# HKUST-Aerial-Robotics/FIESTA

Hardware: AMD Instinct MI355X
Metric: esdf_updated_voxels_per_sec (higher is better)
Workload: dtype u32

## Files before the change

### fiesta_amd/csrc/dense_map.hip

```cpp
#include "dense_map.hpp"
#include "checkpoint.hpp"
#include "frontier_kernels.hpp"
#include "ray_query_kernels.hpp"
#include "reach_kernels.hpp"
#include "reach_matrix_kernels.hpp"
#include "corridor_kernels.hpp"
#include "view_kernels.hpp"
#include "ft_kernels.hpp"
#include "nn_kernels.hpp"
#include "mask_kernels.hpp"
#include "level_kernels.hpp"
#include "path_cost_kernels.hpp"
#include "refine_kernels.hpp"
#include "timing_kernels.hpp"
#include "path_kernels.hpp"
#include "relax_kernels.hpp"

#include <algorithm>
#include <chrono>
#include <cmath>
#include <cstdlib>
#include <cstring>

namespace fiesta {
// ... 1603 lines not shown
  for (int attempt = 0; attempt < 2; ++attempt) {
    cells = attempt == 0 && cells_wanted() && run_cells(st, 0, false);
    if (!cells) {
      bool exact = true;
      if (!run_bulk(st, 0, &exact)) return false;
    }
    const unsigned long long *failed = cells ? &counters_[C_NN_FAILED] : nullptr;
    MaskArgs a = ma;
    a.failed = failed;
    FIESTA_HIP_CHECK(hipEventRecord(ev_cert, stream_));
    hipLaunchKernelGGL(k_mask_classify, dim3(classify_blocks), dim3(256), 0, stream_, a);
    #ifndef FIESTA_WALK_PARTS
#define FIESTA_WALK_PARTS 32
#endif
    hipLaunchKernelGGL(k_mask_walk, dim3(kMaskSegs * FIESTA_WALK_PARTS), dim3(256), 0, stream_, a);
    hipLaunchKernelGGL(k_mask_cells, dim3(std::min(classify_blocks, 1024)), dim3(256), 0, stream_, a);
    FIESTA_HIP_CHECK(hipGetLastError());
    FIESTA_HIP_CHECK(hipEventRecord(ev_rep, stream_));
    gi = 0;
    chain = std::min(std::max(mask_chain_hint_, 2), kMaskIters);
    launch_chain(chain, failed);
    FIESTA_HIP_CHECK(hipEventRecord(ev_end, stream_));
    FIESTA_HIP_CHECK(hipMemcpyAsync(h_mask_ctr_, mask_ctr_, MC_SEG0 * sizeof(unsigned long long), hipMemcpyDeviceToHost, stream_));
    if (cells) FIESTA_HIP_CHECK(hipMemcpyAsync(&h_counters_[C_FT_OVF0], &counters_[C_FT_OVF0], 7 * sizeof(unsigned long long), hipMemcpyDeviceToHost, stream_));
    FIESTA_HIP_CHECK(hipStreamSynchronize(stream_));
#if defined(FIESTA_PROBE)
    fprintf(stderr, "PROBE walks %llu: straight n-sum %llu, steps %llu | paths %llu, positions loaded %llu, refused by cell %llu, n-sum %llu | entries %llu, candidates %llu, none %llu, certified %llu\n",
            h_mask_ctr_[MC_WALKS], h_mask_ctr_[MC_CHANGED0 + 12], h_mask_ctr_[MC_CHANGED0 + 13], h_mask_ctr_[MC_CHANGED0 + 14], h_mask_ctr_[MC_CHANGED0 + 15],
            h_mask_ctr_[MC_CHANGED0 + 16], h_mask_ctr_[MC_CHANGED0 + 17], h_mask_ctr_[MC_CHANGED0 + 18], h_mask_ctr_[MC_CHANGED0 + 19], h_mask_ctr_[MC_CHANGED0 + 20],
            h_mask_ctr_[MC_CHANGED0 + 21]);
#endif
    if (!cells || h_counters_[C_NN_FAILED] == 0) {
      if (cells) nn_fail_streak_ = 0;
      break;
    }
    nn_fail_streak_ = std::min(nn_fail_streak_ + 1, 6);
    nn_skip_ = 4 << nn_fail_streak_;
    const int64_t nfailed = (int64_t)h_counters_[C_NN_FAILED];
    reset_stats_counters(true);
    if (st) {
      memset(&st->cells, 0, sizeof(st->cells));
      st->nn_failed = nfailed;
    }
  }
  float m1 = 0, m2 = 0, m3 = 0, mc = 0, mr = 0;
  (void)hipEventElapsedTime(&m1, ft_ev_[0], ft_ev_[1]);
  (void)hipEventElapsedTime(&m2, ft_ev_[1], ft_ev_[2]);
  (void)hipEventElapsedTime(&m3, ft_ev_[2], ft_ev_[3]);
  (void)hipEventElapsedTime(&mc, ev_cert, ev_rep);
  (void)hipEventElapsedTime(&mr, ev_rep, ev_end);
  if (st)
    for (int k = 0; k < 8; ++k) st->prof[k] = (int64_t)h_mask_ctr_[MC_CHANGED0 + k];
  if (h_mask_ctr_[MC_OVERFLOW] != 0) {
    if (mask_seg_cap_ * kMaskSegs >= (size_t)g.n) return false;
    mask_seg_cap_ *= 2;
    tr_occ_ = nullptr, tr_out_ = nullptr, tr_cellobs_ = nullptr;
    reset_stats_counters(true);
    return run_masked(st);
  }
  int total_iters = 0;
  for (int n = chain;;) {
    int k = 0;
    while (k < n && h_mask_ctr_[MC_CHANGED0 + k] != 0) ++k;
    total_iters += k < n ? k + 1 : n;
    if (k < n || h_mask_ctr_[MC_QUADS] == 0) break;
    FIESTA_HIP_CHECK(hipMemsetAsync(&mask_ctr_[MC_CHANGED0], 0, kMaskIters * sizeof(unsigned long long), stream_));
    FIESTA_HIP_CHECK(hipEventRecord(ev_rep, stream_));
    n = 4;
    launch_chain(n, nullptr);
    FIESTA_HIP_CHECK(hipEventRecord(ev_end, stream_));
    FIESTA_HIP_CHECK(hipMemcpyAsync(&h_mask_ctr_[MC_CHANGED0], &mask_ctr_[MC_CHANGED0], kMaskIters * sizeof(unsigned long long), hipMemcpyDeviceToHost, stream_));
    FIESTA_HIP_CHECK(hipStreamSynchronize(stream_));
    float more = 0;
    (void)hipEventElapsedTime(&more, ev_rep, ev_end);
    mr += more;
  }
  mask_chain_hint_ = std::min(total_iters + 1, kMaskIters);
  std::swap(coc_, mask_out_.p);
  zero_counters(C_INSERT, 2);
  host_counts_[0] = host_counts_[1] = 0;
  queues_zeroed_ = false;
  if (track_) {
    zero_counter(C_MAXD2);
    hipLaunchKernelGGL(k_maxd2_scan, dim3(grid_for(g_.n, 256, 4096)), dim3(256), 0, stream_, g_, (const vox_t *)coc_, counters_);
    FIESTA_HIP_CHECK(hipGetLastError());
  }
  FIESTA_HIP_CHECK(hipEventRecord(ev1_, stream_));
  FIESTA_HIP_CHECK(hipEventSynchronize(ev1_));
  h_counters_fresh_ = false;
  if (cells) nn_last_ms_ = (double)m1 + m2 + m3, nn_last_nocc_ = (long long)h_counters_[C_NOCC];
  else ft_last_ms_ = (double)m1 + m2 + m3;
  if (st) {
    float ms = 0;
    FIESTA_HIP_CHECK(hipEventElapsedTime(&ms, ev0_, ev1_));
    st->device_ms = ms;
    st->bulk = 1, st->cells = cells ? 1 : 0, st->masked = 1;
    if (cells) {
      st->nn_cells_ms = m1, st->nn_lists_ms = m2, st->nn_fill_ms = m3;
      st->nn_entries = (int64_t)h_counters_[C_NN_ENTRIES];
    } else {
      st->ft_rows_ms = m1, st->ft_plane_ms = m2, st->ft_x_ms = m3;
    }
    st->mask_certify_ms = mc, st->mask_repair_ms = mr;
    st->mask_uncertified = (int64_t)h_mask_ctr_[MC_MARKED], st->mask_iterations = total_iters, st->mask_walks = (int64_t)h_mask_ctr_[MC_WALKS];
    st->mask_quads = (int64_t)h_mask_ctr_[MC_QUADS];
    st->relax_ms = (double)m1 + m2 + m3 + mc + mr;
    st->relax_launches = 3 + 3 + 2 * total_iters;
  }
  return true;
}

struct HostMs {
  fiesta_hip_stats *st;
  std::chrono::steady_clock::time_point h0 = std::chrono::steady_clock::now();
  ~HostMs() { if (st) st->host_ms = std::chrono::duration<double, std::milli>(std::chrono::steady_clock::now() - h0).count(); }
};

void DenseMap::bulk_finish(fiesta_hip_stats *st, bool cells, bool published) {
  static_assert(C_DELETE == C_INSERT + 1, "counter layout");
  nn_clean_ = false;
  if (published) {
    FIESTA_HIP_CHECK(hipEventRecord(ev1_, stream_));
    FIESTA_HIP_CHECK(hipEventSynchronize(ev1_));
    published = h_counters_[C_NN_CURSOR] == nn_tag_;
    if (published) {
      h_counters_fresh_ = false;
      if (h_counters_[C_NN_FAILED] == 0) {
        queues_zeroed_ = false;
        host_counts_[0] = host_counts_[1] = 0;
        nn_clean_ = true;
      }
    }
  }
  if (!published) {
    if (!queues_zeroed_) zero_counters(C_INSERT, 2);
    queues_zeroed_ = false;
    host_counts_[0] = host_counts_[1] = 0;
    if (g_.sharded) zero_counter(C_REMOTE_DEL);
    FIESTA_HIP_CHECK(hipEventRecord(ev1_, stream_));
    collect_stats(nullptr);
    FIESTA_HIP_CHECK(hipEventSynchronize(ev1_));
  }
  float m1 = 0, m2 = 0, m3 = 0;
  const bool timed = hipEventElapsedTime(&m1, ft_ev_[0], ft_ev_[1]) == hipSuccess && hipEventElapsedTime(&m2, ft_ev_[1], ft_ev_[2]) == hipSuccess &&
                     hipEventElapsedTime(&m3, ft_ev_[2], ft_ev_[3]) == hipSuccess;
  if (st) {
    float ms = 0;
    FIESTA_HIP_CHECK(hipEventElapsedTime(&ms, ev0_, ev1_));
    st->device_ms = ms;
    if (cells) {
      st->nn_cells_ms = m1, st->nn_lists_ms = m2, st->nn_fill_ms = m3;
      st->nn_entries = (int64_t)h_counters_[C_NN_ENTRIES];
      st->nn_failed = (int64_t)h_counters_[C_NN_FAILED];
      if (st->nn_incremental) st->nn_dirty_cells = (int64_t)h_counters_[C_NN_DIRTY];
      else st->nn_brute_cells = (int64_t)h_counters_[C_NN_BRUTE];
    } else {
      st->ft_rows_ms = m1, st->ft_plane_ms = m2, st->ft_x_ms = m3;
      st->ft_overflow[0] = (int64_t)h_counters_[C_FT_OVF0], st->ft_overflow[3] = (int64_t)h_counters_[C_FT_OVF0 + 3];
    }
    st->relax_ms = (double)m1 + m2 + m3;
  }
  if (cells && published && !(st && st->nn_incremental)) nn_last_brute_ = (long long)h_counters_[C_NN_BRUTE];
  if (timed) {
    if (cells) {
      if (h_counters_[C_NN_FAILED] == 0) nn_last_ms_ = (double)m1 + m2 + m3, nn_last_nocc_ = (long long)h_counters_[C_NOCC];
    } else {
      ft_last_ms_ = (double)m1 + m2 + m3;
    }
  }
}

bool DenseMap::bulk_try(fiesta_hip_stats *st, int margin, bool *exact) {
  ++field_epoch_;
  use_device();
  nn_clean_ = false;
  nn_valid_ = false;
  ++epoch_;
  FIESTA_HIP_CHECK(hipEventRecord(ev0_, stream_));
  reset_stats_counters();
  if (st) memset(st, 0, sizeof(*st));
  tried_cells_ = false;
  if (cells_wanted() && run_cells(st, margin, false)) {
    FIESTA_HIP_CHECK(hipMemcpyAsync(&h_counters_[C_FT_OVF0], &counters_[C_FT_OVF0], 7 * sizeof(unsigned long long), hipMemcpyDeviceToHost, stream_));
    FIESTA_HIP_CHECK(hipStreamSynchronize(stream_));
    if (h_counters_[C_NN_FAILED] == 0) {
      nn_fail_streak_ = 0;
      tried_cells_ = true;
      if (exact) *exact = true;
      if (st) st->ft_max_d2 = (int64_t)h_counters_[C_FT_MAXD2];
      return true;
    }
    cells_back_off();
    const int64_t failed = (int64_t)h_counters_[C_NN_FAILED];
    reset_stats_counters();
    if (st) {
      memset(st, 0, sizeof(*st));
      st->nn_failed = failed;
    }
  }
  return run_bulk(st, margin, exact);
}
void DenseMap::bulk_commit(fiesta_hip_stats *st) {
  ++field_epoch_;
  use_device();
  if (!ft_in_place_) std::swap(coc_, ft_out_.p);
  HostMs host_ms{st};
  bulk_finish(st, tried_cells_);
}
void DenseMap::bulk_probe(unsigned long long *ni, unsigned long long *nd, long long *nocc, bool *eligible) {
  use_device();
  FIESTA_HIP_CHECK(hipMemcpyAsync(&h_counters_[C_INSERT], &counters_[C_INSERT], 4 * sizeof(unsigned long long),
                                  hipMemcpyDeviceToHost, stream_));
  FIESTA_HIP_CHECK(hipStreamSynchronize(stream_));
  for (int k = 0; k < 4; ++k) host_counts_[k] = h_counters_[C_INSERT + k];
  host_counts_valid_ = true;
  *ni = h_counters_[C_INSERT], *nd = h_counters_[C_DELETE];
  *nocc = (long long)h_counters_[C_NOCC];
  *eligible = bulk_eligible(*ni, *nd);
}

void DenseMap::level_tuning(int grid_groups, long long spin_limit) { LevelEngine::tuning(lv_, grid_groups, spin_limit); }
int DenseMap::level_trace(uint32_t *out48) const { return LevelEngine::trace(lv_, out48); }

bool DenseMap::run_levels(fiesta_hip_stats *st, unsigned long long ni, unsigned long long nd) {
  if (!lv_) {
    lv_ = new LevelEngine;
#ifdef FIESTA_HIP_TUNING
    if (const char *e = getenv("FIESTA_HIP_GRID_ENTER")) lv_->grid_enter = (uint32_t)atoi(e);
    if (const char *e = getenv("FIESTA_HIP_GRID_MIN")) lv_->grid_min = (uint32_t)atoi(e);
#endif
  }
  const uint32_t want = update_engine_ == 3 ? (uint32_t)std::min<int64_t>(std::max<int64_t>(g_.n / 4, 1 << 20), 1 << 26) : (1u << 20);
  lv_->ensure(want, stream_);
  LevelUpdate u{};
  u.stream = stream_, u.t0 = ev0_;
  u.coc = coc_, u.counters = counters_, u.track = track_;
  u.ins = (const uint32_t *)ins_.p, u.ni = ni;
  u.scan = nd != 0, u.full_window = g_.full_window();
  u.pinned = update_engine_ == 3, u.tiny = ni + nd <= (unsigned long long)LevelEngine::kTiny;
  u.nwords = g_.n;
  u.tg = TileGrid{tx_, ty_, ntx_, nty_, ntz_}, u.tile_flag = tile_flag_[0], u.tile_list = tile_list_[0], u.list_count = &counters_[C_LIST0];
  const int bounded = (track_ && nd) ? 1 : 0;
  const auto scan = [&](bool levels, const LevelArgs &a) {
    if (levels && bounded) hipLaunchKernelGGL(k_del_bbox, dim3(1), dim3(1024), 0, stream_, g_, (const uint32_t *)del_.p, (int64_t)nd, counters_);
    hipLaunchKernelGGL(levels ? k_invalidate<true> : k_invalidate<false>, dim3((grid_for(g_.n / 16 + 1, 256, 4096) + 7) / 8 * 8), dim3(256), 0,
                       stream_, g_, u.tg, coc_, (const uint32_t *)occbits_, (const uint32_t *)gocc_, tile_flag_[0], tile_list_[0],
                       &counters_[C_LIST0], counters_, bounded, a);
    FIESTA_HIP_CHECK(hipGetLastError());
  };
  host_counts_[0] = host_counts_[1] = 0;
  if (!lv_->update(DenseSpace{g_, occbits_, lv_box(g_)}, u, scan, st)) return false;
  h_counters_fresh_ = false;
  if (st) st->device_ms = st->relax_ms;
  return true;
}

bool DenseMap::serve_by_transform(fiesta_hip_stats *st, unsigned long long ni, unsigned long long nd, bool nn_was_clean, bool nn_was_valid) {
  const bool want_cells = cells_wanted();
  const bool lean = want_cells && nn_was_clean;
  if (lean) {
    queues_zeroed_ = false;
    ft_counters_clean_ = true;
  } else {
    queues_zeroed_ = !g_.sharded && g_.nx <= 2048 && g_.ny <= 2048 && g_.nz <= 2048;
    reset_stats_counters(true, queues_zeroed_);
  }
  const int64_t ncells8 = (int64_t)((g_.nx + 7) / 8) * ((g_.ny + 7) / 8) * ((g_.nz + 7) / 8);
  if (want_cells && nn_was_valid && !g_.wrap && (int64_t)(ni + nd) * 180 <= ncells8 / 2 && run_cells(st, 0, true, true, ni, nd)) {
    bulk_finish(st, true, true);
    if (h_counters_[C_NN_FAILED] == 0) {
      nn_fail_streak_ = 0;
      nn_valid_ = true;
      return true;
    }
    notes_ |= FIESTA_HIP_NOTE_INCREMENTAL_REDONE;
    FIESTA_HIP_CHECK(hipMemsetAsync(nn_dirty_flag_.p, 0, nn_dirty_flag_.cap * sizeof(uint32_t), stream_));
    if (st) memset(&st->cells, 0, sizeof(st->cells)), st->nn_incremental = 0;
    restart_attempt();
  }
  if (want_cells && run_cells(st, 0, true)) {
    bulk_finish(st, true, true);
    if (h_counters_[C_NN_FAILED] == 0) {
      nn_fail_streak_ = 0;
      nn_valid_ = !g_.sharded && h_counters_[C_NN_SPARSE] == 0;
      return true;
    }
    cells_back_off();
    notes_ |= FIESTA_HIP_NOTE_CELLS_FAILED;
    const int64_t failed = (int64_t)h_counters_[C_NN_FAILED];
    if (st) {
      memset(&st->cells, 0, sizeof(st->cells));
      st->nn_failed = failed;
    }
    restart_attempt();
  }
  bool exact = true;
  if (run_bulk(st, 0, &exact)) {
    bulk_finish(st);
    return true;
  }
  if (queues_zeroed_) {
    h_counters_[C_INSERT] = ni, h_counters_[C_DELETE] = nd;
    FIESTA_HIP_CHECK(hipMemcpyAsync(&counters_[C_INSERT], &h_counters_[C_INSERT], 2 * sizeof(unsigned long long), hipMemcpyHostToDevice, stream_));
    queues_zeroed_ = false;
  }
  return false;
// ... 871 lines not shown
```

### fiesta_amd/csrc/nn_kernels.hpp

```cpp
#pragma once
#include "common.hpp"
#include "nn_core.hpp"

namespace fiesta {

struct NnArgs {
  nn::Geom g;
  const uint8_t *cellobs;
  const uint32_t *occ;
  int sx0, sy0, szb;
  int sny, snzw;
  uint32_t *ctab;
  uint32_t *sites;
  uint32_t sites_cap;
  uint32_t *lists;
  unsigned long long *cursor;
  unsigned long long *failed;
  unsigned long long *entries;
  unsigned long long *maxd2;
  vox_t *coc;
  uint32_t *dump;
  unsigned long long *pub, *queues, *track_dst;
  unsigned long long tag;
  int pub_failed, pub_entries, pub_maxd2, pub_tag, pub_dirty, pub_brute, pub_sparse;
// ... 216 lines not shown
    if (rank == 0) (void)atomicExch(counter, 0u);
    __builtin_amdgcn_fence(__ATOMIC_ACQ_REL, "wavefront");
  }
  __device__ __forceinline__ int slot() { return (int)atomicAdd(counter, 1u); }
  __device__ __forceinline__ int count_now() const { return (int)min(atomicAdd(counter, 0u), (uint32_t)nn::kRaw); }
  __device__ __forceinline__ void put(int k, uint32_t v) { raw[k] = v; }
  __device__ __forceinline__ uint32_t get(int k) const { return raw[k]; }
  __device__ __forceinline__ int count() const {
    __builtin_amdgcn_fence(__ATOMIC_ACQ_REL, "wavefront");
    return (int)atomicAdd(counter, 0u);
  }
};

template <bool WRAP>
__global__ __launch_bounds__(1024) __attribute__((amdgpu_waves_per_eu(8, 8))) void k_nn_lists(NnArgs a) {
  __shared__ uint16_t s_tab[kStageNR * kStageNZ];
  __shared__ uint32_t s_first[kStageNR], s_soff[kStageNR], s_cnt[kStageNR];
  __shared__ uint32_t s_sites[kStageSites];
  __shared__ uint32_t s_slots[256];
  __shared__ uint32_t s_raw[256 * (nn::kRaw + 1)];
  __shared__ uint32_t s_total, s_bad, s_sum, s_done;
  __shared__ uint32_t s_te2[256], s_tw[256], s_bin[8];
  __shared__ uint16_t s_order[256];
  __shared__ uint8_t s_key[256];
  const nn::Geom &g = a.g;
  if (*a.failed) return;
  const int tid = (int)threadIdx.x;
  const int cz0 = g.lz0 + (int)blockIdx.x * 64, cy0 = g.ly0 + (int)blockIdx.y * 4, cx = g.lx0 + (int)blockIdx.z;
  const int X0 = cx - kStageK, Y0 = cy0 - kStageK, Zf = cz0 - kStageK;
  const nn::Frame fr = nn::frame_of(g);
  const int64_t rowlen = g.ncz + 1;
  if (tid < 256) s_slots[tid] = 0;
  if (tid == 0) s_bad = 0, s_sum = 0, s_done = 0;
  if (tid < 8) s_bin[tid] = 0;
  if (tid < kStageNR) {
    const int X = X0 + tid / kStageNY, Y = Y0 + tid % kStageNY;
    uint32_t f = 0, l = 0;
    if ((unsigned)X < (unsigned)g.ncx && (unsigned)Y < (unsigned)g.ncy) {
      const uint32_t *row = a.ctab + ((int64_t)X * g.ncy + Y) * rowlen;
      f = row[min(max(Zf, 0), g.ncz)], l = row[min(max(Zf + kStageNZ - 1, 0), g.ncz)];
    }
    s_first[tid] = f, s_cnt[tid] = l - f;
  }
  __syncthreads();
  if (tid < 64) {
    const uint32_t c0 = tid < kStageNR ? s_cnt[tid] : 0u, c1 = tid + 64 < kStageNR ? s_cnt[tid + 64] : 0u;
    uint32_t i0 = c0, i1 = c1;
    for (int off = 1; off < 64; off <<= 1) {
      const uint32_t u0 = (uint32_t)__shfl_up((int)i0, off), u1 = (uint32_t)__shfl_up((int)i1, off);
      if (tid >= off) i0 += u0, i1 += u1;
    }
    const uint32_t t0 = (uint32_t)__shfl((int)i0, 63);
    if (tid < kStageNR) s_soff[tid] = i0 - c0;
    if (tid + 64 < kStageNR) s_soff[tid + 64] = t0 + i1 - c1;
    if (tid == 63) s_total = t0 + i1;
  }
  __syncthreads();
  const bool staged = s_total <= (uint32_t)kStageSites;
  if (staged) {
    for (int idx = tid; idx < kStageNR * kStageNZ; idx += 1024) {
      const int row = idx / kStageNZ, e = idx - row * kStageNZ;
      const int X = X0 + row / kStageNY, Y = Y0 + row % kStageNY;
      uint32_t v = 0;
      if ((unsigned)X < (unsigned)g.ncx && (unsigned)Y < (unsigned)g.ncy)
        v = a.ctab[((int64_t)X * g.ncy + Y) * rowlen + min(max(Zf + e, 0), g.ncz)] - s_first[row];
      s_tab[idx] = (uint16_t)v;
    }
    for (int idx = tid; idx < kStageNR * 16; idx += 1024) {
      const int row = idx >> 4;
      const uint32_t cnt = s_cnt[row], first = s_first[row], at = s_soff[row];
      for (uint32_t j = (uint32_t)(idx & 15); j < cnt; j += 16) s_sites[at + j] = a.sites[first + j];
    }
  }
  __syncthreads();
  const int team_i = tid >> 2;
  QuadTeam team{tid & 3, &s_slots[team_i], &s_raw[team_i * (nn::kRaw + 1)]};
  const StagedSrcT<WRAP> ssrc{staged ? s_tab : nullptr, s_soff, s_sites, -(X0 * kStageNY + Y0), -Zf};
  {
    const int cz = cz0 + (team_i & 63), cy = cy0 + (team_i >> 6);
    const bool live = cz < g.lz1 && cy < g.ly1 && !(a.cellobs && a.cellobs[((int64_t)cx * g.ncy + cy) * g.ncz + cz] == 0);
    int te2 = nn::kNone, key = 7;
    uint32_t tw = 0xFFFFFFFFu;
    if (live) {
      if (staged) nn::first_competitor(ssrc, team, cx, cy, cz, nn::kKfirst, te2, tw);
      key = min(nn::window_reach<WRAP>(te2, tw, cx, cy, cz), 6);
    }
    if (team.rank == 0) {
      s_te2[team_i] = (uint32_t)te2, s_tw[team_i] = tw, s_key[team_i] = (uint8_t)key;
      atomicAdd(&s_bin[key], 1u);
    }
  }
  __syncthreads();
  if (tid == 0) {
    uint32_t at = 0;
    for (int k = 0; k < 8; ++k) {
      const uint32_t c = s_bin[k];
      s_bin[k] = at, at += c;
    }
  }
  __syncthreads();
  if (tid < 256) s_order[atomicAdd(&s_bin[s_key[tid]], 1u)] = (uint16_t)tid;
  __syncthreads();
  const int ci = s_order[team_i];
  const int cz = cz0 + (ci & 63), cy = cy0 + (ci >> 6);
  int n = 0;
  bool live = cz < g.lz1 && cy < g.ly1;
  if (live && a.cellobs && a.cellobs[((int64_t)cx * g.ncy + cy) * g.ncz + cz] == 0) {
    live = false;
    if (team.rank == 0) a.lists[(((int64_t)cx * g.ncy + cy) * g.ncz + cz) * nn::kStride] = 0u;
  }
  if (live) {
    const int64_t cell = ((int64_t)cx * g.ncy + cy) * g.ncz + cz;
    uint32_t *rec = a.lists + cell * nn::kStride;
    n = -1;
    if (staged) n = nn::build_list(ssrc, team, cx, cy, cz, rec, true, (int)s_te2[ci], s_tw[ci], fr);
    if (n < 0) {
      const HybridSrcT<WRAP> src{ssrc, nn::PlainSrcT<WRAP>{a.ctab, a.sites, g.ncx, g.ncy, g.ncz}, X0, Y0, Zf};
      n = nn::build_list(src, team, cx, cy, cz, rec, false, nn::kNone, 0xFFFFFFFFu, fr);
    }
  }
  bool hard = live && team.rank == 0 && n == 0;
  if (hard && a.fail_list && fr.open == 0 && *a.nfail < a.fail_cap) {
    const unsigned long long at = atomicAdd(a.nfail, 1ull);
    if (at < a.fail_cap) {
      a.fail_list[at] = (uint32_t)(((int64_t)cx * g.ncy + cy) * g.ncz + cz);
      hard = false;
    }
  }
  const unsigned long long bad = __ballot(hard);
  int sum = (live && team.rank == 0) ? n : 0;
  for (int off = 32; off > 0; off >>= 1) sum += __shfl_xor(sum, off);
  if ((tid & 63) == 0) {
    if (bad) atomicAdd(&s_bad, (uint32_t)__popcll(bad));
    if (sum) atomicAdd(&s_sum, (uint32_t)sum);
    __threadfence_block();
    if (atomicAdd(&s_done, 1u) == 15u) {
      const uint32_t b = atomicAdd(&s_bad, 0u), t = atomicAdd(&s_sum, 0u);
      if (b) atomicAdd(a.failed, (unsigned long long)b);
      if (t) atomicAdd(a.entries, (unsigned long long)t);
    }
  }
}

__device__ __forceinline__ void nn_dot4_pair(uint32_t a, uint32_t b0, uint32_t b1, int &d0, int &d1) {
  asm("v_dot4_i32_i8 %0, %2, %3, 0\n\tv_dot4_i32_i8 %1, %2, %4, 0\n\ts_nop 2" : "=&v"(d0), "=&v"(d1) : "v"(a), "v"(b0), "v"(b1));
}

#ifndef FIESTA_FILL_BLOCKS
#define FIESTA_FILL_BLOCKS 16384
#endif
constexpr int kFillBlocks = FIESTA_FILL_BLOCKS;
constexpr int kListPad = 256;

template <bool TRACK, bool OFFSET = false>
__global__ __launch_bounds__(256) void k_nn_fill_full(NnArgs a) {
  constexpr int kTileRow = 40;
  __shared__ __attribute__((aligned(16))) uint32_t land[4][2][nn::kStride];
  __shared__ __attribute__((aligned(16))) uint32_t tile[4][nn::kB * kTileRow];
  const nn::Geom &g = a.g;
  if (*a.failed) return;
  const int lane = threadIdx.x & 63, wave = __builtin_amdgcn_readfirstlane((int)(threadIdx.x >> 6));
  const int quads = OFFSET ? (g.lz1 - g.lz0 + 3) >> 2 : g.ncz >> 2;
  const int rows_y = OFFSET ? g.ly1 - g.ly0 : g.ncy;
  const uint32_t nq = (uint32_t)((OFFSET ? g.lx1 - g.lx0 : g.ncx) * rows_y) * (uint32_t)quads;
  const uint32_t per = OFFSET ? (nq + gridDim.x * 4u - 1u) / (gridDim.x * 4u) : nq / (gridDim.x * 4u);
  const uint32_t q0 = (blockIdx.x * 4u + (uint32_t)wave) * per, q1 = OFFSET ? min(q0 + per, nq) : q0 + per;
  if (OFFSET && q0 >= q1) return;
  const int row0 = (int)(q0 / (uint32_t)quads);
  const int y = lane >> 3, z = lane & 7;
  const uint32_t ayz = (uint32_t)y | ((uint32_t)z << 8);
  const int64_t plane = (int64_t)g.ny * g.nz;
  const int loff4 = y * g.nz + 4 * z;
  uint32_t dmax = 0;
  const uint32_t zone0 = (uint32_t)(size_t)&land[wave][0][0];
  uint32_t *const mytile = &tile[wave][0];
  struct At { int cx, cy, q; };
  auto fetch = [&](const At &c, const int cell_of_quad, const int zone) {
    const int64_t cell = OFFSET ? ((int64_t)(g.lx0 + c.cx) * g.ncy + (g.ly0 + c.cy)) * g.ncz + min(g.lz0 + 4 * c.q + cell_of_quad, g.lz1 - 1)
                                : ((int64_t)c.cx * g.ncy + c.cy) * g.ncz + 4 * c.q + cell_of_quad;
    const uint32_t *lp = a.lists + cell * nn::kStride + lane, *hp = lp + 64;
    const uint32_t at = zone0 + (uint32_t)zone * (uint32_t)(nn::kStride * 4);
    asm volatile("s_mov_b32 m0, %0\n\tglobal_load_lds_dword %1, off\n\t"
                 "s_mov_b32 m0, %2\n\tglobal_load_lds_dword %3, off"
                 : : "s"(at), "v"(lp), "s"(at + 256u), "v"(hp) : "memory", "m0");
  };
  auto advance = [&](At &c) {
    if (++c.q == quads) {
      c.q = 0;
      if (++c.cy == rows_y) c.cy = 0, ++c.cx;
    }
  };
  auto serve = [&](const int zone, uint32_t *ww, const bool col_in, const int xin_lo, const int xin_hi) {
    const uint32_t *lz = &land[wave][zone][0];
    const int cnt = __builtin_amdgcn_readfirstlane((int)lz[0]);
    uint32_t best[nn::kB];
#pragma unroll
    for (int x = 0; x < nn::kB; ++x) best[x] = 0xFFFFFFFFu;
    for (int i = 0; i < cnt; i += 2) {
      const uint4 e0 = *reinterpret_cast<const uint4 *>(lz + 4 + 4 * i), e1 = *reinterpret_cast<const uint4 *>(lz + 8 + 4 * i);
      int d0, d1;
      nn_dot4_pair(ayz, e0.x, e1.x, d0, d1);
      uint32_t k0 = ((uint32_t)d0 << nn::kSH) + e0.y, k1 = ((uint32_t)d1 << nn::kSH) + e1.y;
      best[0] = min(best[0], min(k0, k1));
#pragma unroll
      for (int x = 1; x < nn::kB; ++x) {
        k0 += e0.z, k1 += e1.z;
        best[x] = min(best[x], min(k0, k1));
      }
    }
#pragma unroll
    for (int x = 0; x < nn::kB; ++x) {
      ww[x] = *reinterpret_cast<const uint32_t *>(reinterpret_cast<const char *>(lz + 7) + (best[x] & 0x1F0u));
      if (TRACK && (!OFFSET || (col_in && x >= xin_lo && x < xin_hi)))
        dmax = max(dmax, (best[x] >> nn::kSH) - (uint32_t)nn::kBias + (uint32_t)(x * x + y * y + z * z));
    }
  };
  At c{row0 / rows_y, row0 % rows_y, (int)(q0 % (uint32_t)quads)};
  fetch(c, 0, 0);
  asm volatile("s_waitcnt vmcnt(0)" ::: "memory");
  for (uint32_t q = q0; q < q1; ++q) {
    uint32_t ww[4][nn::kB];
    At nxt = c;
    if (q + 1 < q1) advance(nxt);
#pragma unroll
    for (int k = 0; k < 4; ++k) {
      if (k < 3) fetch(c, k + 1, (k + 1) & 1); else fetch(nxt, 0, 0);
      if (k == 0) {
        if (OFFSET) asm volatile("s_waitcnt vmcnt(18)" ::: "memory");
        else asm volatile("s_waitcnt vmcnt(10)" ::: "memory");
      } else {
        asm volatile("s_waitcnt vmcnt(2)" ::: "memory");
      }
      bool col_in = true;
      int xin_lo = 0, xin_hi = nn::kB;
      if (OFFSET && TRACK) {
        const int cz = g.lz0 + 4 * c.q + k;
        const int Y = nn::kB * (g.ly0 + c.cy) + y - g.fy, Z = nn::kB * cz + z - g.fz, X0 = nn::kB * (g.lx0 + c.cx) - g.fx;
        col_in = cz < g.lz1 && (unsigned)Y < (unsigned)g.ay && (unsigned)Z < (unsigned)g.az;
        xin_lo = max(0, -X0), xin_hi = min(nn::kB, g.ax - X0);
      }
      serve(k & 1, ww[k], col_in, xin_lo, xin_hi);
      asm volatile("s_waitcnt lgkmcnt(0)" ::: "memory");
    }
    if (!OFFSET) {
      vox_t *slab = a.coc + ((int64_t)(nn::kB * c.cx) * g.ny + nn::kB * c.cy) * g.nz + 4 * nn::kB * c.q;
#pragma unroll
      for (int x = 0; x < nn::kB; ++x) {
#pragma unroll
        for (int k = 0; k < 4; ++k) mytile[y * kTileRow + nn::kB * k + z] = ww[k][x];
        const uint4 v = *reinterpret_cast<const uint4 *>(&mytile[y * kTileRow + 4 * z]);
        *reinterpret_cast<uint4 *>(slab + loff4) = v;
        slab += plane;
      }
    } else {
      const int srow = lane >> 4, spair = lane & 15;
      const int X0 = nn::kB * (g.lx0 + c.cx) - g.fx, Y0 = nn::kB * (g.ly0 + c.cy) - g.fy;
      const int Zq = nn::kB * (g.lz0 + 4 * c.q) + 2 * spair;
      const bool zin = (unsigned)(Zq - g.fz) < (unsigned)g.az && Zq < nn::kB * g.lz1;
      const int64_t aplane = (int64_t)g.ay * g.az;
      uint32_t *const mydump = a.dump + 2 * lane;
#pragma unroll
      for (int x = 0; x < nn::kB; ++x) {
#pragma unroll
        for (int k = 0; k < 4; ++k) mytile[y * kTileRow + nn::kB * k + z] = ww[k][x];
        const bool xin = (unsigned)(X0 + x) < (unsigned)g.ax;
#pragma unroll
        for (int h = 0; h < 2; ++h) {
          const int r = srow + 4 * h;
          const uint2 v = *reinterpret_cast<const uint2 *>(&mytile[r * kTileRow + 2 * spair]);
          const bool in = xin && zin && (unsigned)(Y0 + r) < (unsigned)g.ay;
          uint32_t *dst = in ? a.coc + (int64_t)(X0 + x) * aplane + (int64_t)(Y0 + r) * g.az + (Zq - g.fz) : mydump;
          *reinterpret_cast<uint2 *>(dst) = v;
        }
      }
    }
    c = nxt;
  }
  if (TRACK) {
    for (int off = 32; off > 0; off >>= 1) dmax = max(dmax, (uint32_t)__shfl_xor((int)dmax, off));
    if (lane == 0 && (unsigned long long)dmax > *a.maxd2) atomicMax(a.maxd2, (unsigned long long)dmax);
  }
}

typedef __attribute__((address_space(4))) const uint32_t nn_cu32;
typedef uint32_t nn_u32x4 __attribute__((ext_vector_type(4)));
typedef __attribute__((address_space(4))) const nn_u32x4 nn_cu32x4;
template <bool TRACK>
__device__ __forceinline__ void nn_fill_cell(const NnArgs &a, const int cx, const int cy, const int cz, const int lane, uint32_t &dmax) {
  const nn::Geom &g = a.g;
  const int64_t cell = ((int64_t)cx * g.ncy + cy) * g.ncz + cz;
  const uint32_t *rec = a.lists + cell * nn::kStride;
  nn_cu32 *lp = reinterpret_cast<nn_cu32 *>(reinterpret_cast<uintptr_t>(rec));
  const int cnt = (int)lp[0];
  const int y = lane >> 3, z = lane & 7;
  const uint32_t ayz = (uint32_t)y | ((uint32_t)z << 8);
  uint32_t best[nn::kB];
#pragma unroll
  for (int x = 0; x < nn::kB; ++x) best[x] = 0xFFFFFFFFu;
  for (int i = 0; i < cnt; ++i) {
    const nn_u32x4 e = *reinterpret_cast<nn_cu32x4 *>(lp + 4 + 4 * i);
    uint32_t k = ((uint32_t)__builtin_amdgcn_sdot4((int)ayz, (int)e.x, 0, false) << nn::kSH) + e.y;
    best[0] = min(best[0], k);
#pragma unroll
    for (int x = 1; x < nn::kB; ++x) {
      k += e.z;
      best[x] = min(best[x], k);
    }
  }
  const int X0 = nn::kB * cx - g.fx, Y = nn::kB * cy + y - g.fy, Z = nn::kB * cz + z - g.fz;
  const bool inyz = (unsigned)Y < (unsigned)g.ay && (unsigned)Z < (unsigned)g.az;
  vox_t *out = a.coc + ((int64_t)X0 * g.ay + Y) * g.az + Z;
  const int64_t plane = (int64_t)g.ay * g.az;
#pragma unroll
  for (int x = 0; x < nn::kB; ++x) {
    const uint32_t ww = rec[7 + ((best[x] & 0x1F0u) >> 2)];
    if (inyz && (unsigned)(X0 + x) < (unsigned)g.ax) {
      out[x * plane] = ww;
      if (TRACK) dmax = max(dmax, (best[x] >> nn::kSH) - (uint32_t)nn::kBias + (uint32_t)(x * x + y * y + z * z));
    }
  }
}

template <bool TRACK>
__global__ __launch_bounds__(256) void k_nn_fill(NnArgs a) {
  const nn::Geom &g = a.g;
  if (*a.failed) return;
  const int lane = threadIdx.x & 63, wave = __builtin_amdgcn_readfirstlane((int)(threadIdx.x >> 6));
  const int cz = g.lz0 + (int)blockIdx.x * 4 + wave, cy = g.ly0 + (int)blockIdx.y, cx = g.lx0 + (int)blockIdx.z;
  if (cz >= g.lz1) return;
  uint32_t dmax = 0;
  nn_fill_cell<TRACK>(a, cx, cy, cz, lane, dmax);
  if (TRACK) {
    for (int off = 32; off > 0; off >>= 1) dmax = max(dmax, (uint32_t)__shfl_xor((int)dmax, off));
    if (lane == 0 && (unsigned long long)dmax > *a.maxd2) atomicMax(a.maxd2, (unsigned long long)dmax);
  }
}

constexpr int kMarkQueue = 4096;
__global__ __launch_bounds__(1024) void k_nn_mark(NnArgs a) {
  __shared__ uint32_t s_q[kMarkQueue];
  __shared__ uint32_t s_n;
  __shared__ unsigned long long s_base;
  const nn::Geom &g = a.g;
  const uint32_t total = a.nchg[0] + a.nchg[1];
  constexpr int E = 2 * nn::kKmax + 1, E3 = E * E * E;
  const unsigned long long pairs = (unsigned long long)total * E3;
  if (threadIdx.x == 0) s_n = 0;
  __syncthreads();
  for (unsigned long long p0 = (unsigned long long)blockIdx.x * blockDim.x; p0 < pairs; p0 += (unsigned long long)gridDim.x * blockDim.x) {
    const unsigned long long p = p0 + threadIdx.x;
    if (p < pairs) {
      const uint32_t v = (uint32_t)(p / E3);
      const int o = (int)(p - (unsigned long long)v * E3);
      const uint32_t idx = v < a.nchg[0] ? a.chg[0][v] : a.chg[1][v - a.nchg[0]];
      const int z = (int)(idx % (uint32_t)g.nz), y = (int)((idx / (uint32_t)g.nz) % (uint32_t)g.ny), x = (int)(idx / ((uint32_t)g.nz * (uint32_t)g.ny));
      const int dz = o % E - nn::kKmax, dy = (o / E) % E - nn::kKmax, dx = o / (E * E) - nn::kKmax;
      const int cx = (x >> 3) + dx, cy = (y >> 3) + dy, cz = (z >> 3) + dz;
      if ((unsigned)cx < (unsigned)g.ncx && (unsigned)cy < (unsigned)g.ncy && (unsigned)cz < (unsigned)g.ncz) {
        const int64_t c = ((int64_t)cx * g.ncy + cy) * g.ncz + cz;
        const int r = max(max(dx < 0 ? -dx : dx, dy < 0 ? -dy : dy), dz < 0 ? -dz : dz);
        if (r <= (int)(a.lists[c * nn::kStride + 1] & 255u) && a.dirty_flag[c] == 0u && atomicExch(&a.dirty_flag[c], 1u) == 0u)
          s_q[atomicAdd(&s_n, 1u)] = (uint32_t)c;
      }
    }
    __syncthreads();
    const uint32_t n = s_n;
    const bool last = p0 + (unsigned long long)gridDim.x * blockDim.x >= pairs;
    if (n && (last || n > (uint32_t)kMarkQueue - 1024u)) {
      if (threadIdx.x == 0) s_base = atomicAdd(a.dirty_count, (unsigned long long)n);
      __syncthreads();
      const unsigned long long base = s_base;
      for (uint32_t i = threadIdx.x; i < n; i += blockDim.x)
        if (base + i < a.dirty_cap) a.dirty_list[base + i] = s_q[i];
      __syncthreads();
      if (threadIdx.x == 0) s_n = 0;
    }
    __syncthreads();
  }
}

__global__ __launch_bounds__(256) void k_nn_lists_dirty(NnArgs a) {
  __shared__ uint32_t s_slots[16];
  __shared__ uint32_t s_raw[16 * (nn::kRaw + 1)];
  const nn::Geom &g = a.g;
  if (*a.failed) return;
  const unsigned long long nd = *a.dirty_count;
  if (nd > a.dirty_cap) {
    if (blockIdx.x == 0 && threadIdx.x == 0) atomicAdd(a.failed, 1ull);
    return;
  }
  const int tid = (int)threadIdx.x, team_i = tid >> 4;
  const nn::Frame fr = nn::frame_of(g);
  const nn::PlainSrcT<false> src{a.ctab, a.sites, g.ncx, g.ncy, g.ncz};
  unsigned bad = 0, entries = 0;
  for (unsigned long long i = blockIdx.x * 16ull + (unsigned long long)team_i; i < nd; i += gridDim.x * 16ull) {
    const uint32_t c = a.dirty_list[i];
    const int cz = (int)(c % (uint32_t)g.ncz), cy = (int)((c / (uint32_t)g.ncz) % (uint32_t)g.ncy), cx = (int)(c / ((uint32_t)g.ncz * (uint32_t)g.ncy));
    WideTeam team{tid & 15, &s_slots[team_i], &s_raw[team_i * (nn::kRaw + 1)]};
    if (team.rank == 0) s_slots[team_i] = 0;
    __builtin_amdgcn_fence(__ATOMIC_ACQ_REL, "wavefront");
    const int n = nn::build_list(src, team, cx, cy, cz, a.lists + (int64_t)c * nn::kStride, false, nn::kNone, 0xFFFFFFFFu, fr);
    if (team.rank == 0) {
      if (n <= 0) ++bad; else entries += (unsigned)n;
    }
  }
  for (int off = 32; off > 0; off >>= 1) {
    bad += (unsigned)__shfl_xor((int)bad, off);
    entries += (unsigned)__shfl_xor((int)entries, off);
  }
  if ((tid & 63) == 0) {
    if (bad) atomicAdd(a.failed, (unsigned long long)bad);
    (void)entries;
  }
}

template <bool TRACK>
__global__ __launch_bounds__(256) void k_nn_fill_dirty(NnArgs a) {
  const nn::Geom &g = a.g;
  if (*a.failed) return;
  const unsigned long long nd = *a.dirty_count;
  const int lane = threadIdx.x & 63, wave = __builtin_amdgcn_readfirstlane((int)(threadIdx.x >> 6));
  uint32_t dmax = 0;
  for (unsigned long long i = blockIdx.x * 4ull + (unsigned long long)wave; i < nd; i += gridDim.x * 4ull) {
    const uint32_t c = a.dirty_list[i];
    const int cz = (int)(c % (uint32_t)g.ncz), cy = (int)((c / (uint32_t)g.ncz) % (uint32_t)g.ncy), cx = (int)(c / ((uint32_t)g.ncz * (uint32_t)g.ncy));
    nn_fill_cell<TRACK>(a, cx, cy, cz, lane, dmax);
    if (lane == 0) a.dirty_flag[c] = 0u;
  }
  if (TRACK) {
    for (int off = 32; off > 0; off >>= 1) dmax = max(dmax, (uint32_t)__shfl_xor((int)dmax, off));
    if (lane == 0 && (unsigned long long)dmax > *a.maxd2) atomicMax(a.maxd2, (unsigned long long)dmax);
  }
}

// ... 104 lines not shown
```

Before: 8.038 billion.

## Fetch NN list records by count-sized lines instead of whole records in fill

Splits the non-offset full fill kernel into a separate path that loads each cell's candidate list into LDS in 128-byte lines. The first line of all four cells in a quad is prefetched one quad ahead, a second line is fetched only when the count exceeds 7, and the whole record is loaded synchronously only when it exceeds 15. The aim is to cut global-to-LDS traffic for cells with short lists. In exchange it adds count-dependent branching, a serialized wait on the rare long-list path, and a second LDS buffer per wave. It also records the tracked max d2 in stats for the NN path.

```diff
diff --git a/fiesta_amd/csrc/dense_map.hip b/fiesta_amd/csrc/dense_map.hip
--- a/fiesta_amd/csrc/dense_map.hip
+++ b/fiesta_amd/csrc/dense_map.hip
@@ -1779,6 +1779,7 @@
       st->nn_cells_ms = m1, st->nn_lists_ms = m2, st->nn_fill_ms = m3;
       st->nn_entries = (int64_t)h_counters_[C_NN_ENTRIES];
       st->nn_failed = (int64_t)h_counters_[C_NN_FAILED];
+      if (published && track_) st->ft_max_d2 = (int64_t)h_counters_[C_FT_MAXD2];
       if (st->nn_incremental) st->nn_dirty_cells = (int64_t)h_counters_[C_NN_DIRTY];
       else st->nn_brute_cells = (int64_t)h_counters_[C_NN_BRUTE];
     } else {
diff --git a/fiesta_amd/csrc/nn_kernels.hpp b/fiesta_amd/csrc/nn_kernels.hpp
--- a/fiesta_amd/csrc/nn_kernels.hpp
+++ b/fiesta_amd/csrc/nn_kernels.hpp
@@ -392,32 +392,149 @@
 constexpr int kFillBlocks = FIESTA_FILL_BLOCKS;
 constexpr int kListPad = 256;
 
-template <bool TRACK, bool OFFSET = false>
-__global__ __launch_bounds__(256) void k_nn_fill_full(NnArgs a) {
+template <bool TRACK>
+__device__ __forceinline__ void nn_fill_full_lines(const NnArgs &a) {
   constexpr int kTileRow = 40;
-  __shared__ __attribute__((aligned(16))) uint32_t land[4][2][nn::kStride];
+  constexpr int kSlot = 64;
+  __shared__ __attribute__((aligned(16))) uint32_t land[4][2][4][kSlot];
+  __shared__ __attribute__((aligned(16))) uint32_t whole[4][nn::kStride];
   __shared__ __attribute__((aligned(16))) uint32_t tile[4][nn::kB * kTileRow];
   const nn::Geom &g = a.g;
   if (*a.failed) return;
   const int lane = threadIdx.x & 63, wave = __builtin_amdgcn_readfirstlane((int)(threadIdx.x >> 6));
-  const int quads = OFFSET ? (g.lz1 - g.lz0 + 3) >> 2 : g.ncz >> 2;
-  const int rows_y = OFFSET ? g.ly1 - g.ly0 : g.ncy;
-  const uint32_t nq = (uint32_t)((OFFSET ? g.lx1 - g.lx0 : g.ncx) * rows_y) * (uint32_t)quads;
-  const uint32_t per = OFFSET ? (nq + gridDim.x * 4u - 1u) / (gridDim.x * 4u) : nq / (gridDim.x * 4u);
-  const uint32_t q0 = (blockIdx.x * 4u + (uint32_t)wave) * per, q1 = OFFSET ? min(q0 + per, nq) : q0 + per;
-  if (OFFSET && q0 >= q1) return;
+  const int quads = g.ncz >> 2;
+  const uint32_t nq = (uint32_t)(g.ncx * g.ncy) * (uint32_t)quads;
+  const uint32_t per = nq / (gridDim.x * 4u);
+  const uint32_t q0 = (uint32_t)__builtin_amdgcn_readfirstlane((int)((blockIdx.x * 4u + (uint32_t)wave) * per)), q1 = q0 + per;
   const int row0 = (int)(q0 / (uint32_t)quads);
   const int y = lane >> 3, z = lane & 7;
   const uint32_t ayz = (uint32_t)y | ((uint32_t)z << 8);
   const int64_t plane = (int64_t)g.ny * g.nz;
   const int loff4 = y * g.nz + 4 * z;
+  const uint32_t lane4 = 4u * (uint32_t)lane;
+  uint32_t dmax = 0;
+  const uint32_t set0 = (uint32_t)(size_t)&land[wave][0][0][0];
+  const uint32_t whole0 = (uint32_t)(size_t)&whole[wave][0];
+  uint32_t *const mytile = &tile[wave][0];
+  const char *const recs = reinterpret_cast<const char *>(a.lists);
+  auto quad_recs = [&](const uint32_t q) { return recs + (uint64_t)q * (uint64_t)(4 * nn::kStride * 4); };
+  auto fetch_lines = [&](const char *p0, const char *p1, const char *p2, const char *p3, const uint32_t at) {
+    if (lane < 32)
+      asm volatile("s_mov_b32 m0, %5\n\ts_nop 0\n\tglobal_load_lds_dword %0, %1\n\t"
+                   "s_mov_b32 m0, %6\n\ts_nop 0\n\tglobal_load_lds_dword %0, %2\n\t"
+                   "s_mov_b32 m0, %7\n\ts_nop 0\n\tglobal_load_lds_dword %0, %3\n\t"
+                   "s_mov_b32 m0, %8\n\ts_nop 0\n\tglobal_load_lds_dword %0, %4"
+                   : : "v"(lane4), "s"(p0), "s"(p1), "s"(p2), "s"(p3), "s"(at), "s"(at + 256u), "s"(at + 512u), "s"(at + 768u)
+                   : "memory", "m0");
+  };
+  auto fetch_line0 = [&](const char *qr, const int set) {
+    fetch_lines(qr, qr + 512, qr + 1024, qr + 1536, set0 + (uint32_t)set * (uint32_t)(4 * kSlot * 4));
+  };
+  auto fetch_line1 = [&](const char *qr, const int set, const int *cnt) {
+    fetch_lines(qr + (cnt[0] > 7 ? 128 : 0), qr + 512 + (cnt[1] > 7 ? 128 : 0), qr + 1024 + (cnt[2] > 7 ? 128 : 0),
+                qr + 1536 + (cnt[3] > 7 ? 128 : 0), set0 + (uint32_t)set * (uint32_t)(4 * kSlot * 4) + 128u);
+  };
+  auto fetch_whole = [&](const char *qr, const int k) {
+    asm volatile("s_mov_b32 m0, %3\n\ts_nop 0\n\tglobal_load_lds_dword %0, %1\n\t"
+                 "s_mov_b32 m0, %4\n\ts_nop 0\n\tglobal_load_lds_dword %0, %2\n\t"
+                 "s_waitcnt vmcnt(0)"
+                 : : "v"(lane4), "s"(qr + 512 * k), "s"(qr + 512 * k + 256), "s"(whole0), "s"(whole0 + 256u) : "memory", "m0");
+  };
+  auto serve = [&](const uint32_t *lz, const int cnt, uint32_t *ww) {
+    uint32_t best[nn::kB];
+#pragma unroll
+    for (int x = 0; x < nn::kB; ++x) best[x] = 0xFFFFFFFFu;
+    for (int i = 0; i < cnt; i += 2) {
+      const int j = i + 1 < cnt ? i + 1 : i;
+      const uint4 e0 = *reinterpret_cast<const uint4 *>(lz + 4 + 4 * i), e1 = *reinterpret_cast<const uint4 *>(lz + 4 + 4 * j);
+      int d0, d1;
+      nn_dot4_pair(ayz, e0.x, e1.x, d0, d1);
+      uint32_t k0 = ((uint32_t)d0 << nn::kSH) + e0.y, k1 = ((uint32_t)d1 << nn::kSH) + e1.y;
+      best[0] = min(best[0], min(k0, k1));
+#pragma unroll
+      for (int x = 1; x < nn::kB; ++x) {
+        k0 += e0.z, k1 += e1.z;
+        best[x] = min(best[x], min(k0, k1));
+      }
+    }
+#pragma unroll
+    for (int x = 0; x < nn::kB; ++x) {
+      ww[x] = *reinterpret_cast<const uint32_t *>(reinterpret_cast<const char *>(lz + 7) + (best[x] & 0x1F0u));
+      if (TRACK) dmax = max(dmax, (best[x] >> nn::kSH) - (uint32_t)nn::kBias + (uint32_t)(x * x + y * y + z * z));
+    }
+  };
+  struct At { int cx, cy, q; };
+  At c{row0 / g.ncy, row0 % g.ncy, (int)(q0 % (uint32_t)quads)};
+  fetch_line0(quad_recs(q0), 0);
+  for (uint32_t q = q0; q < q1; ++q) {
+    if (q == q0) asm volatile("s_waitcnt vmcnt(0)" ::: "memory");
+    else asm volatile("s_waitcnt vmcnt(8)" ::: "memory");
+    const int set = (int)((q - q0) & 1u);
+    const uint32_t *const slots = &land[wave][set][0][0];
+    const char *const qr = quad_recs(q);
+    int cnt[4];
+#pragma unroll
+    for (int k = 0; k < 4; ++k)
+      cnt[k] = min(__builtin_amdgcn_readfirstlane((int)slots[k * kSlot]), nn::kCap);
+    asm volatile("s_waitcnt lgkmcnt(0)" ::: "memory");
+    fetch_line1(qr, set, cnt);
+    fetch_line0(quad_recs(q + 1 < q1 ? q + 1 : q), set ^ 1);
+    uint32_t ww[4][nn::kB];
+#pragma unroll
+    for (int k = 0; k < 4; ++k) {
+      const uint32_t *lz = slots + k * kSlot;
+      if (cnt[k] > 15) {
+        fetch_whole(qr, k);
+        lz = &whole[wave][0];
+      } else if (cnt[k] > 7) {
+        asm volatile("s_waitcnt vmcnt(4)" ::: "memory");
+      }
+      serve(lz, cnt[k], ww[k]);
+      asm volatile("s_waitcnt lgkmcnt(0)" ::: "memory");
+    }
+    vox_t *slab = a.coc + ((int64_t)(nn::kB * c.cx) * g.ny + nn::kB * c.cy) * g.nz + 4 * nn::kB * c.q;
+#pragma unroll
+    for (int x = 0; x < nn::kB; ++x) {
+#pragma unroll
+      for (int k = 0; k < 4; ++k) mytile[y * kTileRow + nn::kB * k + z] = ww[k][x];
+      const uint4 v = *reinterpret_cast<const uint4 *>(&mytile[y * kTileRow + 4 * z]);
+      *reinterpret_cast<uint4 *>(slab + loff4) = v;
+      slab += plane;
+    }
+    if (++c.q == quads) {
+      c.q = 0;
+      if (++c.cy == g.ncy) c.cy = 0, ++c.cx;
+    }
+  }
+  if (TRACK) {
+    for (int off = 32; off > 0; off >>= 1) dmax = max(dmax, (uint32_t)__shfl_xor((int)dmax, off));
+    if (lane == 0 && (unsigned long long)dmax > *a.maxd2) atomicMax(a.maxd2, (unsigned long long)dmax);
+  }
+}
+
+template <bool TRACK>
+__device__ __forceinline__ void nn_fill_full_offset(const NnArgs &a) {
+  constexpr int kTileRow = 40;
+  __shared__ __attribute__((aligned(16))) uint32_t land[4][2][nn::kStride];
+  __shared__ __attribute__((aligned(16))) uint32_t tile[4][nn::kB * kTileRow];
+  const nn::Geom &g = a.g;
+  if (*a.failed) return;
+  const int lane = threadIdx.x & 63, wave = __builtin_amdgcn_readfirstlane((int)(threadIdx.x >> 6));
+  const int quads = (g.lz1 - g.lz0 + 3) >> 2;
+  const int rows_y = g.ly1 - g.ly0;
+  const uint32_t nq = (uint32_t)((g.lx1 - g.lx0) * rows_y) * (uint32_t)quads;
+  const uint32_t per = (nq + gridDim.x * 4u - 1u) / (gridDim.x * 4u);
+  const uint32_t q0 = (blockIdx.x * 4u + (uint32_t)wave) * per, q1 = min(q0 + per, nq);
+  if (q0 >= q1) return;
+  const int row0 = (int)(q0 / (uint32_t)quads);
+  const int y = lane >> 3, z = lane & 7;
+  const uint32_t ayz = (uint32_t)y | ((uint32_t)z << 8);
   uint32_t dmax = 0;
   const uint32_t zone0 = (uint32_t)(size_t)&land[wave][0][0];
   uint32_t *const mytile = &tile[wave][0];
   struct At { int cx, cy, q; };
   auto fetch = [&](const At &c, const int cell_of_quad, const int zone) {
-    const int64_t cell = OFFSET ? ((int64_t)(g.lx0 + c.cx) * g.ncy + (g.ly0 + c.cy)) * g.ncz + min(g.lz0 + 4 * c.q + cell_of_quad, g.lz1 - 1)
-                                : ((int64_t)c.cx * g.ncy + c.cy) * g.ncz + 4 * c.q + cell_of_quad;
+    const int64_t cell = ((int64_t)(g.lx0 + c.cx) * g.ncy + (g.ly0 + c.cy)) * g.ncz + min(g.lz0 + 4 * c.q + cell_of_quad, g.lz1 - 1);
     const uint32_t *lp = a.lists + cell * nn::kStride + lane, *hp = lp + 64;
     const uint32_t at = zone0 + (uint32_t)zone * (uint32_t)(nn::kStride * 4);
     asm volatile("s_mov_b32 m0, %0\n\tglobal_load_lds_dword %1, off\n\t"
@@ -451,7 +568,7 @@
 #pragma unroll
     for (int x = 0; x < nn::kB; ++x) {
       ww[x] = *reinterpret_cast<const uint32_t *>(reinterpret_cast<const char *>(lz + 7) + (best[x] & 0x1F0u));
-      if (TRACK && (!OFFSET || (col_in && x >= xin_lo && x < xin_hi)))
+      if (TRACK && col_in && x >= xin_lo && x < xin_hi)
         dmax = max(dmax, (best[x] >> nn::kSH) - (uint32_t)nn::kBias + (uint32_t)(x * x + y * y + z * z));
     }
   };
@@ -465,15 +582,11 @@
 #pragma unroll
     for (int k = 0; k < 4; ++k) {
       if (k < 3) fetch(c, k + 1, (k + 1) & 1); else fetch(nxt, 0, 0);
-      if (k == 0) {
-        if (OFFSET) asm volatile("s_waitcnt vmcnt(18)" ::: "memory");
-        else asm volatile("s_waitcnt vmcnt(10)" ::: "memory");
-      } else {
-        asm volatile("s_waitcnt vmcnt(2)" ::: "memory");
-      }
+      if (k == 0) asm volatile("s_waitcnt vmcnt(18)" ::: "memory");
+      else asm volatile("s_waitcnt vmcnt(2)" ::: "memory");
       bool col_in = true;
       int xin_lo = 0, xin_hi = nn::kB;
-      if (OFFSET && TRACK) {
+      if (TRACK) {
         const int cz = g.lz0 + 4 * c.q + k;
         const int Y = nn::kB * (g.ly0 + c.cy) + y - g.fy, Z = nn::kB * cz + z - g.fz, X0 = nn::kB * (g.lx0 + c.cx) - g.fx;
         col_in = cz < g.lz1 && (unsigned)Y < (unsigned)g.ay && (unsigned)Z < (unsigned)g.az;
@@ -482,36 +595,24 @@
       serve(k & 1, ww[k], col_in, xin_lo, xin_hi);
       asm volatile("s_waitcnt lgkmcnt(0)" ::: "memory");
     }
-    if (!OFFSET) {
-      vox_t *slab = a.coc + ((int64_t)(nn::kB * c.cx) * g.ny + nn::kB * c.cy) * g.nz + 4 * nn::kB * c.q;
-#pragma unroll
-      for (int x = 0; x < nn::kB; ++x) {
-#pragma unroll
-        for (int k = 0; k < 4; ++k) mytile[y * kTileRow + nn::kB * k + z] = ww[k][x];
-        const uint4 v = *reinterpret_cast<const uint4 *>(&mytile[y * kTileRow + 4 * z]);
-        *reinterpret_cast<uint4 *>(slab + loff4) = v;
-        slab += plane;
-      }
-    } else {
-      const int srow = lane >> 4, spair = lane & 15;
-      const int X0 = nn::kB * (g.lx0 + c.cx) - g.fx, Y0 = nn::kB * (g.ly0 + c.cy) - g.fy;
-      const int Zq = nn::kB * (g.lz0 + 4 * c.q) + 2 * spair;
-      const bool zin = (unsigned)(Zq - g.fz) < (unsigned)g.az && Zq < nn::kB * g.lz1;
-      const int64_t aplane = (int64_t)g.ay * g.az;
-      uint32_t *const mydump = a.dump + 2 * lane;
-#pragma unroll
-      for (int x = 0; x < nn::kB; ++x) {
-#pragma unroll
-        for (int k = 0; k < 4; ++k) mytile[y * kTileRow + nn::kB * k + z] = ww[k][x];
-        const bool xin = (unsigned)(X0 + x) < (unsigned)g.ax;
-#pragma unroll
-        for (int h = 0; h < 2; ++h) {
-          const int r = srow + 4 * h;
-          const uint2 v = *reinterpret_cast<const uint2 *>(&mytile[r * kTileRow + 2 * spair]);
-          const bool in = xin && zin && (unsigned)(Y0 + r) < (unsigned)g.ay;
-          uint32_t *dst = in ? a.coc + (int64_t)(X0 + x) * aplane + (int64_t)(Y0 + r) * g.az + (Zq - g.fz) : mydump;
-          *reinterpret_cast<uint2 *>(dst) = v;
-        }
+    const int srow = lane >> 4, spair = lane & 15;
+    const int X0 = nn::kB * (g.lx0 + c.cx) - g.fx, Y0 = nn::kB * (g.ly0 + c.cy) - g.fy;
+    const int Zq = nn::kB * (g.lz0 + 4 * c.q) + 2 * spair;
+    const bool zin = (unsigned)(Zq - g.fz) < (unsigned)g.az && Zq < nn::kB * g.lz1;
+    const int64_t aplane = (int64_t)g.ay * g.az;
+    uint32_t *const mydump = a.dump + 2 * lane;
+#pragma unroll
+    for (int x = 0; x < nn::kB; ++x) {
+#pragma unroll
+      for (int k = 0; k < 4; ++k) mytile[y * kTileRow + nn::kB * k + z] = ww[k][x];
+      const bool xin = (unsigned)(X0 + x) < (unsigned)g.ax;
+#pragma unroll
+      for (int h = 0; h < 2; ++h) {
+        const int r = srow + 4 * h;
+        const uint2 v = *reinterpret_cast<const uint2 *>(&mytile[r * kTileRow + 2 * spair]);
+        const bool in = xin && zin && (unsigned)(Y0 + r) < (unsigned)g.ay;
+        uint32_t *dst = in ? a.coc + (int64_t)(X0 + x) * aplane + (int64_t)(Y0 + r) * g.az + (Zq - g.fz) : mydump;
+        *reinterpret_cast<uint2 *>(dst) = v;
       }
     }
     c = nxt;
@@ -520,6 +621,12 @@
     for (int off = 32; off > 0; off >>= 1) dmax = max(dmax, (uint32_t)__shfl_xor((int)dmax, off));
     if (lane == 0 && (unsigned long long)dmax > *a.maxd2) atomicMax(a.maxd2, (unsigned long long)dmax);
   }
+}
+
+template <bool TRACK, bool OFFSET = false>
+__global__ __launch_bounds__(256) void k_nn_fill_full(NnArgs a) {
+  if constexpr (OFFSET) nn_fill_full_offset<TRACK>(a);
+  else nn_fill_full_lines<TRACK>(a);
 }
 
 typedef __attribute__((address_space(4))) const uint32_t nn_cu32;
```

Result: no change. 8.005 billion (-0.4%).
